# MpokiAbel/UPMEM--OpenFHE

Hardware: AMD Instinct MI355X
Metric: 64-bit coeffs/sec for NTT+Hadamard+INTT, N=2^16, 16 towers; % HBM roofline (higher is better)
Workload: dtype u64; 1 GPU; configs[2]: N=2^16, towers=16, batch=1024 per GPU, c = INTT(NTT(a) (.) b); log_n=16, towers=16, batch_per_gpu=1024, global_batch=1024, parallelism=batch-sharded x1 (no data-path collective)

## Files before the change

### upmem--openfhe_amd/csrc/ntt_kernels.hpp

```cpp
#pragma once
#include "arith.hpp"

namespace ofhe {

struct TowerConst {
    u64 q;
    u64 ninv;
    u64 ninv_pre;
    u64 mu;
    u64 nq;
    u64 nq4;
    u32 nshift;
    u32 spq_sh;
    u64 qinv;
    u32 one;
    u32 pad_;
};
template <bool SPQ>
__device__ __forceinline__ Mod<SPQ> load_mod(const TowerConst& tc) {
    return Mod<SPQ>{tc.q, 4 * tc.q, 8 * tc.q, tc.nq, tc.nq4, 0 - 8 * tc.q, tc.spq_sh, tc.one};
}

struct PlanArgs {
    const TowerConst* tc;
    const u64* tw;
    const u64* itw;
    const u64* tw3;
    u64 sstride;
    u64 dstride;
    u64 bstride;
    const u64* scal;
    const u64* dtw;
    const u64* twist;
    u32 log_n;
    u32 towers;
};

enum { MODE_FWD = 0, MODE_INV = 1, MODE_FUSED = 2, MODE_FWD_SUB = 3 };

__device__ __forceinline__ u32 xcd_remap(u32 bid, u32 nwg) {
    u32 q = nwg >> 3, r = nwg & 7, xcd = bid & 7, loc = bid >> 3;
    return (xcd < r ? xcd * (q + 1) : r * (q + 1) + (xcd - r) * q) + loc;
}

struct Tw {
    u64 w, wp;
};

typedef u64 u64x2 __attribute__((ext_vector_type(2)));
__device__ __forceinline__ u64 ld_s(const u64* p) { return __builtin_nontemporal_load(p); }
__device__ __forceinline__ void st_s(u64* p, u64 v) { __builtin_nontemporal_store(v, p); }
__device__ __forceinline__ u64x2 ld2_s(const u64* p) {
    return __builtin_nontemporal_load(reinterpret_cast<const u64x2*>(p));
}
__device__ __forceinline__ void st2_s(u64* p, u64x2 v) { __builtin_nontemporal_store(v, reinterpret_cast<u64x2*>(p)); }
__device__ __forceinline__ Tw ldtw(const u64* base, u32 idx) {
    const ulonglong2 v = *reinterpret_cast<const ulonglong2*>(base + 2 * (u64)idx);
    return Tw{v.x, v.y};
}

template <bool SPQ, bool QA>
__device__ __forceinline__ u64 red16(u64 x, const Mod<SPQ, QA>& M) {
    if (SPQ) return fold_spq(x, M);
    return csub_s(x, M.q8);
}
template <bool SPQ, bool QA>
__device__ __forceinline__ void ct_bfly_cs(u64& x, u64& y, Tw w, const Mod<SPQ, QA>& M, bool cs) {
    const u64 a = cs ? red16(x, M) : x;
    x = shoup_lazy_acc(y, w.w, w.wp, M, a);
    y = (a << 1) + M.q4 - x;
}
template <int CS, class M_>
__device__ __forceinline__ void ct_bfly(u64& x, u64& y, Tw w, const M_& M) {
    ct_bfly_cs(x, y, w, M, CS != 0);
}

template <bool SPQ, bool QA>
__device__ __forceinline__ u64 red8(u64 x, const Mod<SPQ, QA>& M) {
    return csub_s(x, M.q4);
}
template <bool SPQ, bool QA>
__device__ __forceinline__ u64 red16_gs(u64 x, const Mod<SPQ, QA>& M) {
    return csub_s(x, M.q8);
}

template <class M_>
__device__ __forceinline__ void gs_bfly(u64& x, u64& y, Tw w, const M_& M) {
    const u64 s = x + y;
    const u64 d = x + M.q4 - y;
    x = red8(s, M);
    y = shoup_lazy(d, w.w, w.wp, M);
}

__device__ __forceinline__ u64 canon8(u64 x, u64 q) {
    x = csub_s(x, 4 * q);
    x = csub_s(x, 2 * q);
    return csub_s(x, q);
}
__device__ __forceinline__ u64 canon4(u64 x, u64 q) {
    x = csub_s(x, 2 * q);
    return csub_s(x, q);
}
template <bool SPQ, bool QA>
__device__ __forceinline__ u64 canon_spq(u64 x, const Mod<SPQ, QA>& M) {
    const u32 qh = hi32(x) >> M.sh;
    const u64 d = (1ull << (M.sh + 32)) - M.q;
    const u64 xm = pack(lo32(x), hi32(x) & ((1u << M.sh) - 1));
    return csub_s(mad32(qh, lo32(d), xm), M.q);
}
template <bool SPQ, bool QA>
__device__ __forceinline__ u64 canon8m(u64 x, const Mod<SPQ, QA>& M) {
    return SPQ ? canon_spq(x, M) : canon8(x, M.q);
}
template <bool SPQ, bool QA>
__device__ __forceinline__ u64 canon4m(u64 x, const Mod<SPQ, QA>& M) {
    return SPQ ? canon_spq(x, M) : canon4(x, M.q);
}
template <bool SPQ, bool QA>
__device__ __forceinline__ u64 canon_fwd(u64 x, const Mod<SPQ, QA>& M) {
    if (SPQ) return canon_spq(x, M);
    const u64 q = M.q;
    x = csub_s(x, 8 * q);
    return canon8(x, q);
}


__device__ __forceinline__ void triv_bfly(u64& x, u64& y, u64 bq) {
    const u64 s = x + y;
    y = x + bq - y;
    x = s;
}

template <int H, int CS, class M_>
__device__ __forceinline__ void dit_stage16(u64 (&v)[16], const u64* base, u32 st, const M_& M) {
    constexpr int half = 1 << H;
#pragma unroll
    for (int j = 0; j < half; j++) {
        const Tw w = ldtw(base, st * j);
#pragma unroll
        for (int g = 0; g < 16; g += 2 * half) ct_bfly<CS>(v[g + j], v[g + j + half], w, M);
    }
}
template <class M_>
__device__ __forceinline__ void dit_round16(u64 (&v)[16], const u64* dtw, u32 st, u32 r, const M_& M) {
    dit_stage16<0, 1>(v, dtw + 2 * ((u64)st + r), st, M);
    dit_stage16<1, 0>(v, dtw + 2 * ((u64)2 * st + r), st, M);
    dit_stage16<2, 1>(v, dtw + 2 * ((u64)4 * st + r), st, M);
    dit_stage16<3, 0>(v, dtw + 2 * ((u64)8 * st + r), st, M);
}

template <bool SPQ, bool QA>
__device__ __forceinline__ void dit_round3(u64 (&v)[16], const u64* dtw, const Mod<SPQ, QA>& M) {
#pragma unroll
    for (int g = 0; g < 16; g += 2) triv_bfly(v[g], v[g + 1], 2 * M.q);
#pragma unroll
    for (int g = 0; g < 16; g += 4) triv_bfly(v[g], v[g + 2], M.q4);
    {
        const Tw w = ldtw(dtw, 3);
#pragma unroll
        for (int g = 0; g < 16; g += 4) ct_bfly<0>(v[g + 1], v[g + 3], w, M);
    }
#pragma unroll
    for (int g = 0; g < 16; g += 8) triv_bfly(v[g], v[g + 4], M.q8);
#pragma unroll
    for (int j = 1; j < 4; j++) {
        const Tw w = ldtw(dtw, 4 + j);
#pragma unroll
        for (int g = 0; g < 16; g += 8) ct_bfly<0>(v[g + j], v[g + j + 4], w, M);
    }
    {
        const u64 a = red16(v[0], M), b = red16(v[8], M);
        v[0] = a;
        v[8] = b;
        triv_bfly(v[0], v[8], M.q8);
    }
#pragma unroll
    for (int j = 1; j < 8; j++) ct_bfly<1>(v[j], v[j + 8], ldtw(dtw, 8 + j), M);
}

template <bool SPQ, bool QA>
__device__ __forceinline__ u64 twist_out(u64 x, Tw f, const Mod<SPQ, QA>& M) {
    return canon4m(shoup_lazy(x, f.w, f.wp, M), M);
}

template <int S, class M_, int CS = S & 1>
__device__ __forceinline__ void fwd_stage16(u64 (&v)[16], const u64* tw, u32 M0, const M_& M) {
    constexpr int half = 8 >> S;
    const u64* base = tw + 2 * ((u64)M0 << S);
#pragma unroll
    for (int j = 0; j < (1 << S); j++) {
        Tw w = ldtw(base, j);
#pragma unroll
        for (int k = j * 2 * half; k < j * 2 * half + half; k++) ct_bfly<CS>(v[k], v[k + half], w, M);
    }
}

template <int S, class M_>
__device__ __forceinline__ void inv_stage16(u64 (&v)[16], const u64* itw, u32 M0, const M_& M) {
    constexpr int half = 8 >> S;
    const u64* base = itw + 2 * ((u64)M0 << S);
#pragma unroll
    for (int j = 0; j < (1 << S); j++) {
        Tw w = ldtw(base, j);
#pragma unroll
        for (int k = j * 2 * half; k < j * 2 * half + half; k++) gs_bfly(v[k], v[k + half], w, M);
    }
}

template <class M_>
__device__ __forceinline__ void gs_bfly_b(u64& x, u64& y, Tw w, const M_& M, bool in8) {
    const u64 s = x + y;
    const u64 d = x + (in8 ? M.q8 : M.q4) - y;
    x = in8 ? red16_gs(s, M) : s;
    y = shoup_lazy(d, w.w, w.wp, M);
}
template <int S, class M_>
__device__ __forceinline__ void inv_stage16_b(u64 (&v)[16], bool (&b8)[16], const u64* itw, u32 M0, const M_& M) {
    constexpr int half = 8 >> S;
    const u64* base = itw + 2 * ((u64)M0 << S);
#pragma unroll
    for (int j = 0; j < (1 << S); j++) {
        Tw w = ldtw(base, j);
#pragma unroll
        for (int k = j * 2 * half; k < j * 2 * half + half; k++) {
            gs_bfly_b(v[k], v[k + half], w, M, b8[k] || b8[k + half]);
            b8[k] = true;
            b8[k + half] = false;
        }
    }
}
template <class M_>
__device__ __forceinline__ void inv_round16_b(u64 (&v)[16], bool (&b8)[16], const u64* itw, u32 M0, const M_& M) {
    inv_stage16_b<3>(v, b8, itw, M0, M);
    inv_stage16_b<2>(v, b8, itw, M0, M);
    inv_stage16_b<1>(v, b8, itw, M0, M);
    inv_stage16_b<0>(v, b8, itw, M0, M);
}

template <class M_>
__device__ __forceinline__ void fwd_round16(u64 (&v)[16], const u64* tw, u32 M0, const M_& M) {
    fwd_stage16<0>(v, tw, M0, M);
    fwd_stage16<1>(v, tw, M0, M);
    fwd_stage16<2>(v, tw, M0, M);
    fwd_stage16<3>(v, tw, M0, M);
}
template <class M_>
__device__ __forceinline__ void fwd_round16_canon(u64 (&v)[16], const u64* tw, u32 M0, const M_& M) {
    fwd_stage16<0>(v, tw, M0, M);
    fwd_stage16<1, M_, 0>(v, tw, M0, M);
    fwd_stage16<2>(v, tw, M0, M);
    fwd_stage16<3>(v, tw, M0, M);
}
template <class M_>
__device__ __forceinline__ void inv_round16(u64 (&v)[16], const u64* itw, u32 M0, const M_& M) {
    inv_stage16<3>(v, itw, M0, M);
    inv_stage16<2>(v, itw, M0, M);
    inv_stage16<1>(v, itw, M0, M);
    inv_stage16<0>(v, itw, M0, M);
}

template <int S, class M_>
__device__ __forceinline__ void fwd_stage16_t3(u64 (&v)[16], const u64* tw3, u32 U, u32 u, const M_& M) {
    constexpr int half = 8 >> S;
    const u64* base = tw3 + 2 * (u64)(((1u << S) - 1) * U);
#pragma unroll
    for (int j = 0; j < (1 << S); j++) {
        Tw w = ldtw(base + 2 * (u64)j * U, u);
#pragma unroll
        for (int k = j * 2 * half; k < j * 2 * half + half; k++) ct_bfly<S & 1>(v[k], v[k + half], w, M);
    }
}
__device__ __forceinline__ u32 lds_pad(u32 p) { return p + (p >> 4); }
constexpr u32 LDS_WORDS = 4096 + 4096 / 16;

template <bool TEAM>
struct StageMap {
    u32 l, base;
    static constexpr u32 E = TEAM ? 32 : 128;
    __device__ __forceinline__ explicit StageMap(u32 tid)
        : l(TEAM ? (tid & 15) : (tid & 63)), base(TEAM ? (tid >> 4) * 256 : (tid >> 6) * 1024) {}
    __device__ __forceinline__ u32 g(int k) const { return E * k + 2 * l; }
    __device__ __forceinline__ u32 p(int k) const { return lds_pad(base + g(k)); }
};
template <bool TEAM>
__device__ __forceinline__ void wave_stage_in(const u64* wsrc, u64* lds, u32 tid, u64 (&out)[16]) {
    const StageMap<TEAM> m(tid);
#pragma unroll
    for (int k = 0; k < 8; k++) {
        const u64x2 v = ld2_s(wsrc + m.g(k));
        lds[m.p(k)] = v.x;
        lds[m.p(k) + 1] = v.y;
    }
    __builtin_amdgcn_wave_barrier();
#pragma unroll
    for (int k = 0; k < 16; k++) out[k] = lds[tid * 17 + k];
    __builtin_amdgcn_wave_barrier();
}
template <bool TEAM, int NPRE>
__device__ __forceinline__ void wave_stage_in_pre(const u64* wsrc, u64* lds, u32 tid, const u64x2 (&pre)[NPRE > 0 ? NPRE : 1],
                                                  u64 (&out)[16]) {
    const StageMap<TEAM> m(tid);
#pragma unroll
    for (int k = 0; k < 8; k++) {
        const u64x2 v = k < NPRE ? pre[k < NPRE ? k : 0] : ld2_s(wsrc + m.g(k));
        lds[m.p(k)] = v.x;
        lds[m.p(k) + 1] = v.y;
    }
    __builtin_amdgcn_wave_barrier();
#pragma unroll
    for (int k = 0; k < 16; k++) out[k] = lds[tid * 17 + k];
    __builtin_amdgcn_wave_barrier();
}
template <bool TEAM>
__device__ __forceinline__ void wave_stage_out(const u64 (&v)[16], u64* lds, u32 tid, u64* wdst, bool live = true) {
    const StageMap<TEAM> m(tid);
#pragma unroll
    for (int k = 0; k < 16; k++) lds[tid * 17 + k] = v[k];
    __builtin_amdgcn_wave_barrier();
    u64x2 w[8];
#pragma unroll
    for (int k = 0; k < 8; k++) {
        w[k].x = lds[m.p(k)];
        w[k].y = lds[m.p(k) + 1];
    }
    if (live) {
#pragma unroll
        for (int k = 0; k < 8; k++) st2_s(wdst + m.g(k), w[k]);
    }
}

#ifndef OFHE_B_PF
#define OFHE_B_PF 8
#endif
#ifndef OFHE_KB_WAVES
#define OFHE_KB_WAVES 4
#endif
template <int NR>
__device__ __forceinline__ void block_sync() {
    if (NR == 2)
        __builtin_amdgcn_wave_barrier();
    else
        __syncthreads();
}
template <int MODE, bool SPQ, int NR, int SK = 0>
__device__ __forceinline__ void block_body(const PlanArgs& P, const u64* src, u64* dst, const u64* __restrict__ bdat,
                                           u32 batch, u32 wid, u64* lds, u32 tid) {
    static_assert(NR == 2 || NR == 3, "k_block covers the last 8 (NR=2) or 12 (NR=3) stages");
    static_assert(SK == 0 || (SK == 3 && NR == 3), "k_block: SK = 3 needs NR = 3");
    constexpr bool TEAM = NR == 2;
    const u32 logn = P.log_n;
    const u32 N = 1u << logn;
    const u32 h = tid >> 4, r = tid & 15;
    u32 g, t, b;
    bool live = true;
    if (TEAM) {
        const u32 G4 = N >> 10, nq = (batch + 3) >> 2;
        const u32 wave = __builtin_amdgcn_readfirstlane(tid >> 6);
        g = (wid % G4) * 4 + wave;
        const u32 pq = wid / G4;
        t = pq / nq;
        const u32 bt = (pq % nq) * 4 + (h & 3);
        live = bt < batch;
        b = live ? bt : batch - 1;
    } else {
        const u32 G = N >> 12;
        g = wid % G;
        const u32 pb = wid / G;
        t = pb / batch;
        b = pb % batch;
    }
    const u64 inner = (u64)t * N + ((u64)g << (TEAM ? 8 : 12));
    const u64 off = (u64)b * P.dstride + inner;
    const u64 boff = (u64)b * P.bstride + inner;
    const u32 wq = TEAM ? 0 : (tid >> 6) * 1024;
    const u64* blk = src + (u64)b * P.sstride + inner;
    u64* oblk = dst + off;
    const TowerConst tc = P.tc[t];
    const u64 q = tc.q;
    const Mod<SPQ> M = load_mod<SPQ>(tc);
    const u64* tw = P.tw + (u64)t * N * 2;
    const u32 L1 = tid + h;
    const u32 L2 = h * 272 + r;
    const u32 L3 = tid * 17;
    u64 v[16];

    if (MODE == MODE_FWD || MODE == MODE_FUSED || MODE == MODE_FWD_SUB) {
        if (NR == 3) {
#pragma unroll
            for (int k = 0; k < 16; k++) v[k] = ld_s(blk + tid + 256 * k);
            if (SK == 3)
                fwd_stage16<3>(v, tw, (N >> 12) + g, M);
            else
                fwd_round16(v, tw, (N >> 12) + g, M);
#pragma unroll
            for (int k = 0; k < 16; k++) lds[L1 + 272 * k] = v[k];
            __syncthreads();
#pragma unroll
            for (int k = 0; k < 16; k++) v[k] = lds[L2 + 17 * k];
        } else {
#pragma unroll
            for (int k = 0; k < 16; k++) v[k] = ld_s(blk + r + 16 * k);
        }
        fwd_round16(v, tw, (N >> 8) + (TEAM ? g : g * 16 + h), M);
#pragma unroll
        for (int k = 0; k < 16; k++) lds[L2 + 17 * k] = v[k];
        block_sync<NR>();
#pragma unroll
        for (int k = 0; k < 16; k++) v[k] = lds[L3 + k];
        constexpr int BPF = (MODE == MODE_FUSED || MODE == MODE_FWD_SUB) ? OFHE_B_PF : 0;
        u64x2 bpre[BPF > 0 ? BPF : 1];
#pragma unroll
        for (int k = 0; k < BPF; k++) bpre[k] = ld2_s(bdat + boff + wq + StageMap<TEAM>(tid).g(k));
        {
            const u64* tw3 = P.tw3 + (u64)t * (N / 16) * 30;
            const u32 U = N >> 4, u = TEAM ? g * 16 + r : g * 256 + tid;
            fwd_stage16_t3<0>(v, tw3, U, u, M);
            fwd_stage16_t3<1>(v, tw3, U, u, M);
            fwd_stage16_t3<2>(v, tw3, U, u, M);
            fwd_stage16_t3<3>(v, tw3, U, u, M);
        }
        if (MODE == MODE_FWD) {
#pragma unroll
            for (int k = 0; k < 16; k++) v[k] = canon_fwd<SPQ>(v[k], M);
            wave_stage_out<TEAM>(v, lds, tid, oblk + wq, live);
            return;
        }
        if (MODE == MODE_FWD_SUB) {
            u64 xx[16];
            wave_stage_in_pre<TEAM, BPF>(bdat + boff + wq, lds, tid, bpre, xx);
            const u64 sc = P.scal[3 * t + 1], scp = P.scal[3 * t + 2];
            const u64 q12 = M.q8 + M.q4;
#pragma unroll
            for (int k = 0; k < 16; k++) v[k] = canon4m(shoup_lazy(xx[k] + q12 - v[k], sc, scp, M), M);
            wave_stage_out<TEAM>(v, lds, tid, oblk + wq, live);
            return;
        }
        u64 bb[16];
        wave_stage_in_pre<TEAM, BPF>(bdat + boff + wq, lds, tid, bpre, bb);
#pragma unroll
        for (int k = 0; k < 16; k++) v[k] = mont_mul(v[k], bb[k], q, tc.qinv);
    } else {
        wave_stage_in<TEAM>(blk + wq, lds, tid, v);
    }
    const u64* dtw = P.dtw + (u64)t * N * 2;
    dit_round3(v, dtw, M);
#pragma unroll
    for (int k = 0; k < 16; k++) lds[L3 + k] = v[k];
    block_sync<NR>();
#pragma unroll
    for (int k = 0; k < 16; k++) v[k] = lds[L2 + 17 * k];
    dit_round16(v, dtw, 16, r, M);
    const u64* tw_ = P.twist + (u64)t * N * 2 + 2 * ((u64)g << (TEAM ? 8 : 12));
    if (NR == 2) {
#pragma unroll
        for (int k = 0; k < 16; k++) {
            const Tw f = ldtw(tw_, r + 16 * k);
            v[k] = shoup_lazy(v[k], f.w, f.wp, M);
        }
        if (live) {
#pragma unroll
            for (int k = 0; k < 16; k++) st_s(oblk + r + 16 * k, v[k]);
        }
        return;
    }
#pragma unroll
    for (int k = 0; k < 16; k++) lds[L2 + 17 * k] = v[k];
    __syncthreads();
#pragma unroll
    for (int k = 0; k < 16; k++) v[k] = lds[L1 + 272 * k];
    if (SK == 3)
        dit_stage16<0, 1>(v, dtw + 2 * ((u64)256 + tid), 256, M);
    else
        dit_round16(v, dtw, 256, tid, M);
#pragma unroll
    for (int k = 0; k < 16; k++) {
        const Tw f = ldtw(tw_, tid + 256 * k);
        v[k] = logn == 12 ? twist_out(v[k], f, M) : shoup_lazy(v[k], f.w, f.wp, M);
    }
#pragma unroll
    for (int k = 0; k < 16; k++) st_s(oblk + tid + 256 * k, v[k]);
}
template <int MODE, bool SPQ, int NR, int SK = 0>
__global__ __launch_bounds__(256, OFHE_KB_WAVES) void k_block(PlanArgs P, const u64* src, u64* dst,
                                                              const u64* __restrict__ bdat, u32 batch, u32 nwg) {
    OFHE_VGPR_FLOOR();
    __shared__ u64 lds[LDS_WORDS];
    block_body<MODE, SPQ, NR, SK>(P, src, dst, bdat, batch, xcd_remap(blockIdx.x, nwg), lds, threadIdx.x);
}

struct SwSrc {
    const u64* last;
    u64 lstride;
    u64 ql;
    const u64* tab;
    u64 pre, pre_p;
};
#ifndef OFHE_TCOLS_W
#define OFHE_TCOLS_W 16
#endif
constexpr u32 TCOLS_W = OFHE_TCOLS_W;
static_assert(TCOLS_W == 16 || TCOLS_W == 32, "column tile width");
constexpr u32 TCOLS_LDS_WORDS = 16 * 16 * TCOLS_W + 16 * 16;
template <bool INV, bool SPQ, bool SWS = false, int LOGN = 16>
__device__ __forceinline__ void tcols_body(const PlanArgs& P, const u64* src, u64* dst, u32 batch, u32 wid,
                                           const SwSrc& SWA, u64* lds, u32 tid) {
    static_assert(LOGN == 16 || LOGN == 17, "k_tcols: N = 2^16 or 2^17");
    constexpr u32 N = 1u << LOGN, S = N / 256, W = TCOLS_W;
    const u32 cb = wid % (S / W);
    const u32 pb = wid / (S / W);
    const u32 t = pb / batch, b = pb % batch;
    const u64 inner = (u64)t * N + cb * W;
    const u64* x = src + (u64)b * P.sstride + inner;
    u64* y = dst + (u64)b * P.dstride + inner;
    const TowerConst tc = P.tc[t];
    const Mod<SPQ> M = load_mod<SPQ>(tc);
    const u32 h = tid / W, r = tid % W;
    const u32 L1 = tid, L2 = h * 16 * W + r;
    u64 v[16];
    if (!INV) {
        const u64* tw = P.tw + (u64)t * N * 2;
        constexpr u32 RP = 16 * W + 16;
        if (SWS) {
            const u64 w = SWA.tab[6 * t + 1], wp = SWA.tab[6 * t + 2];
            const SwMod sm = sw_mod(SWA.ql, tc.q);
            const u64* lp = SWA.last + (u64)b * SWA.lstride + cb * W;
#pragma unroll
            for (int k = 0; k < 16; k++) {
                u64 e = lp[(u64)(h + 16 * k) * S + r];
                if (SWA.pre != 1) e = shoup_canon(e, SWA.pre, SWA.pre_p, SWA.ql);
                e = switch_mod1(e, sm);
                v[k] = w != 1 ? shoup_canon(e, w, wp, tc.q) : e;
            }
        } else {
#pragma unroll
            for (int k = 0; k < 16; k++) v[k] = ld_s(x + (u64)(h + 16 * k) * S + r);
        }
        fwd_round16_canon(v, tw, 1, M);
#pragma unroll
        for (int k = 0; k < 16; k++) lds[L1 + RP * k] = v[k];
        __syncthreads();
#pragma unroll
        for (int k = 0; k < 16; k++) v[k] = lds[h * RP + r + W * k];
        fwd_round16(v, tw, 16 + h, M);
#pragma unroll
        for (int k = 0; k < 16; k++) st_s(y + (u64)(16 * h + k) * S + r, v[k]);
    } else {
        const u64* itw = P.itw + (u64)t * N * 2;
#pragma unroll
        for (int k = 0; k < 16; k++) v[k] = ld_s(x + (u64)(16 * h + k) * S + r);
        bool b8[16];
#pragma unroll
        for (int k = 0; k < 16; k++) b8[k] = false;
        inv_round16_b(v, b8, itw, 16 + h, M);
#pragma unroll
        for (int k = 0; k < 16; k++) lds[L2 + W * k] = v[k];
        __syncthreads();
#pragma unroll
        for (int k = 0; k < 16; k++) {
            v[k] = lds[L1 + 16 * W * k];
            b8[k] = true;
        }
        inv_round16_b(v, b8, itw, 1, M);
#pragma unroll
        for (int k = 0; k < 16; k++)
            st_s(y + (u64)(h + 16 * k) * S + r, b8[k] ? canon8m(v[k], M) : canon4m(v[k], M));
    }
}

template <bool INV, bool SPQ, bool SWS = false, int LOGN = 16>
__global__ __launch_bounds__(16 * TCOLS_W, OFHE_KB_WAVES) void k_tcols(PlanArgs P, const u64* src, u64* dst, u32 batch,
                                                                       u32 nwg, SwSrc SWA) {
    OFHE_VGPR_FLOOR();
    __shared__ u64 lds[TCOLS_LDS_WORDS];
    tcols_body<INV, SPQ, SWS, LOGN>(P, src, dst, batch, xcd_remap(blockIdx.x, nwg), SWA, lds, threadIdx.x);
}

template <bool INV, bool SPQ>
__global__ __launch_bounds__(512) void k_tcols9(PlanArgs P, const u64* src, u64* dst, u32 batch, u32 nwg) {
    OFHE_VGPR_FLOOR();
    constexpr u32 N = 1u << 17, S = 256, W = 16, HALF = 16 * 16 * W;
    __shared__ u64 lds[2 * HALF];
    const u32 tid = threadIdx.x;
    const u32 hf = tid >> 8, tl = tid & 255;
    const u32 wid = xcd_remap(blockIdx.x, nwg);
    const u32 cb = wid % (S / W);
    const u32 pb = wid / (S / W);
    const u32 t = pb / batch, b = pb % batch;
    const u64 inner = (u64)t * N + (u64)hf * 256 * S + cb * W;
    const u64* x = src + (u64)b * P.sstride + inner;
    u64* y = dst + (u64)b * P.dstride + inner;
    const TowerConst tc = P.tc[t];
    const Mod<SPQ> M = load_mod<SPQ>(tc);
    const u32 h = tl / W, r = tl % W;
    u64* my = lds + hf * HALF;
    const u64* other = lds + (hf ^ 1) * HALF;
    const u32 L1 = tl, L2 = h * 16 * W + r;
    u64 v[16];
    if (!INV) {
        const u64* tw = P.tw + (u64)t * N * 2;
#pragma unroll
        for (int k = 0; k < 16; k++) v[k] = ld_s(x + (u64)(h + 16 * k) * S + r);
        const Tw w1 = ldtw(tw, 1);
        if (hf) {
#pragma unroll
            for (int k = 0; k < 16; k++) v[k] = shoup_lazy(v[k], w1.w, w1.wp, M);
        }
#pragma unroll
        for (int k = 0; k < 16; k++) my[L1 + 16 * W * k] = v[k];
        __syncthreads();
        if (hf) {
#pragma unroll
            for (int k = 0; k < 16; k++) v[k] = other[L1 + 16 * W * k] + M.q4 - v[k];
        } else {
#pragma unroll
            for (int k = 0; k < 16; k++) v[k] += other[L1 + 16 * W * k];
        }
        __syncthreads();
        fwd_round16(v, tw, 2 + hf, M);
#pragma unroll
        for (int k = 0; k < 16; k++) my[L1 + 16 * W * k] = v[k];
        __syncthreads();
#pragma unroll
        for (int k = 0; k < 16; k++) v[k] = my[L2 + W * k];
        fwd_round16(v, tw, 32 + 16 * hf + h, M);
#pragma unroll
        for (int k = 0; k < 16; k++) st_s(y + (u64)(16 * h + k) * S + r, v[k]);
    } else {
        const u64* itw = P.itw + (u64)t * N * 2;
#pragma unroll
        for (int k = 0; k < 16; k++) v[k] = ld_s(x + (u64)(16 * h + k) * S + r);
        inv_round16(v, itw, 32 + 16 * hf + h, M);
#pragma unroll
        for (int k = 0; k < 16; k++) my[L2 + W * k] = v[k];
        __syncthreads();
#pragma unroll
        for (int k = 0; k < 16; k++) v[k] = my[L1 + 16 * W * k];
        inv_round16(v, itw, 2 + hf, M);
#pragma unroll
        for (int k = 0; k < 16; k++) my[L1 + 16 * W * k] = v[k];
        __syncthreads();
// ... 184 lines not shown
```

### upmem--openfhe_amd/csrc/ofhe_hip.hip

```cpp
#include <cstdio>
#include <cstdlib>
#include <cstring>
#include <new>
#include <thread>

#include "compose.hpp"
#include "bconv_cols.hpp"

using namespace ofhe;

#define OFHE_VERSION "ofhe-hip 0.2 gfx950"

namespace ofhe {
static thread_local std::string g_err;
int fail(int code, const std::string& msg) {
    g_err = msg;
    return code;
}
int post_launch() {
    hipError_t e = hipGetLastError();
    if (e != hipSuccess) return fail(OFHE_ERR_HIP, std::string("kernel launch: ") + hipGetErrorString(e));
    return OFHE_OK;
}
}
// ... 348 lines not shown
                  {(void**)&p->d_itw, itw.data(), words(itw)},
                  {(void**)&p->d_tw3, tw3.data(), words(tw3)},
                  {(void**)&p->d_dtw, dtw.data(), words(dtw)},
                  {(void**)&p->d_twist, twist.data(), words(twist)},
                  {(void**)&p->d_twist_r, twist_r.data(), words(twist_r)}};
    int rc = OFHE_OK;
    for (const auto& t : tables)
        if (rc == OFHE_OK) rc = alloc_upload(t.dst, t.src, t.bytes, "plan upload", ctx->device);
    if (rc != OFHE_OK) {
        ofhe_hip_plan_destroy(p);
        return rc;
    }
    *plan = p;
    return OFHE_OK;
}

int ofhe_hip_plan_tune(ofhe_plan_t p, uint32_t chunk_batch, uint32_t streams) {
    if (!p || !p->ctx) return fail(OFHE_ERR_STATE, "plan is NULL or destroyed");
    if (streams < 1 || streams > 2) return fail(OFHE_ERR_ARG, "streams must be 1 or 2");
    HIPCHK(hipSetDevice(p->ctx->device));
    std::lock_guard<std::mutex> lk(p->fork_mu);
    if (streams == 2 && !p->st[0]) {
        hipStream_t st[2] = {nullptr, nullptr};
        hipEvent_t fork = nullptr, join[2] = {nullptr, nullptr};
        hipError_t e = hipSuccess;
        for (int i = 0; i < 2 && e == hipSuccess; i++) {
            e = hipStreamCreateWithFlags(&st[i], hipStreamNonBlocking);
            if (e == hipSuccess) e = hipEventCreateWithFlags(&join[i], hipEventDisableTiming);
        }
        if (e == hipSuccess) e = hipEventCreateWithFlags(&fork, hipEventDisableTiming);
        if (e != hipSuccess) {
            for (int i = 0; i < 2; i++) {
                if (st[i]) (void)hipStreamDestroy(st[i]);
                if (join[i]) (void)hipEventDestroy(join[i]);
            }
            if (fork) (void)hipEventDestroy(fork);
            return fail(OFHE_ERR_HIP, std::string("plan_tune: ") + hipGetErrorString(e));
        }
        for (int i = 0; i < 2; i++) {
            p->st[i] = st[i];
            p->ev_join[i] = join[i];
        }
        p->ev_fork = fork;
    }
    p->chunk_batch = chunk_batch;
    p->nstreams = streams;
    return OFHE_OK;
}

int ofhe_hip_plan_destroy(ofhe_plan_t p) {
    if (!p) return fail(OFHE_ERR_ARG, "plan is NULL");
    if (p->ctx) (void)hipSetDevice(p->ctx->device);
    for (int i = 0; i < 2; i++) {
        if (p->st[i]) (void)hipStreamSynchronize(p->st[i]);
        if (p->st[i]) (void)hipStreamDestroy(p->st[i]);
        if (p->ev_join[i]) (void)hipEventDestroy(p->ev_join[i]);
    }
    if (p->ev_fork) (void)hipEventDestroy(p->ev_fork);
    (void)hipFree(p->d_tc);
    (void)hipFree(p->d_tw);
    (void)hipFree(p->d_itw);
    (void)hipFree(p->d_tw3);
    (void)hipFree(p->d_dtw);
    (void)hipFree(p->d_twist);
    (void)hipFree(p->d_twist_r);
    for (auto& kv : p->tabs) (void)hipFree(kv.second);
    delete p;
    return OFHE_OK;
}

int ofhe_hip_plan_tables(ofhe_plan_t p, uint64_t* tab, uint64_t* tab_pre, uint64_t* itab,
                         uint64_t* itab_pre, uint64_t* ninv) {
    if (!p) return fail(OFHE_ERR_ARG, "plan is NULL");
    const size_t n = p->tab.size() * sizeof(u64);
    if (tab) memcpy(tab, p->tab.data(), n);
    if (tab_pre) memcpy(tab_pre, p->tab_pre.data(), n);
    if (itab) memcpy(itab, p->itab.data(), n);
    if (itab_pre) memcpy(itab_pre, p->itab_pre.data(), n);
    if (ninv) memcpy(ninv, p->ninv.data(), p->ninv.size() * sizeof(u64));
    return OFHE_OK;
}

static PlanArgs args_of(ofhe_plan_t p, u32 t0 = 0, u32 count = 0) {
    if (!count) count = p->towers - t0;
    const u64 N = 1ull << p->log_n;
    PlanArgs a;
    a.tc = p->d_tc + t0;
    a.tw = p->d_tw + 2 * N * t0;
    a.itw = p->d_itw + 2 * N * t0;
    a.tw3 = p->d_tw3 + (N >= 4096 ? (N / 16) * 30 * t0 : 0);
    a.sstride = a.dstride = a.bstride = N * count;
    a.scal = nullptr;
    a.dtw = p->d_dtw + 2 * N * t0;
    a.twist = p->d_twist + 2 * N * t0;
    a.log_n = p->log_n;
    a.towers = count;
    return a;
}

static PlanArgs fused_args(ofhe_plan_t p) {
    PlanArgs a = args_of(p);
    if (p->log_n >= 12) a.twist = p->d_twist_r;
    return a;
}

static int check_common(ofhe_plan_t p, uint32_t batch) {
    if (!p || !p->ctx) return fail(OFHE_ERR_STATE, "plan is NULL or destroyed");
    if (batch == 0) return fail(OFHE_ERR_ARG, "batch must be >= 1");
    const u64 polys = (u64)batch * p->towers;
    if (polys * ((u64)1 << p->log_n) / 4096 >= (1ull << 31))
        return fail(OFHE_ERR_ARG, "batch too large for one launch");
    return OFHE_OK;
}

#ifndef OFHE_COLS_CPT
#define OFHE_COLS_CPT 2
#endif
static void launch_colpass(const PlanArgs& a, bool spq, int split, bool inv, const u64* src, u64* dst, u32 batch,
                           hipStream_t s, const SwSrc* lift = nullptr) {
    const SwSrc S = lift ? *lift : SwSrc{nullptr, 0, 0, nullptr, 1, 0};
    const u32 polys = batch * a.towers;
    with_bool(spq, [&](auto sp) { with_bool(inv, [&](auto iv) { with_bool(lift != nullptr, [&](auto sw) {
        constexpr bool SP = decltype(sp)::value, INV = decltype(iv)::value, SWS = decltype(sw)::value;
        if constexpr (!(INV && SWS)) {
            if (split == SPLIT_T9) {
                if constexpr (!SWS) {
                    const u32 nwg = polys * 16;
                    hipLaunchKernelGGL((k_tcols9<INV, SP>), dim3(nwg), dim3(512), 0, s, a, src, dst, batch, nwg);
                }
            } else if (split != SPLIT_COLS) {
                with_int<16, 17>(split == SPLIT_T8B9 ? 17 : 16, [&](auto ln) {
                    constexpr int LOGN = decltype(ln)::value;
                    const u32 nwg = polys * ((1u << (LOGN - 8)) / TCOLS_W);
                    hipLaunchKernelGGL((k_tcols<INV, SP, SWS, LOGN>), dim3(nwg), dim3(16 * TCOLS_W), 0, s, a, src,
                                       dst, batch, nwg, S);
                });
            } else {
                with_int<1, 2, 3, 4, 5>((int)a.log_n - 12, [&](auto ka) {
                    constexpr int KA = decltype(ka)::value, CPT = KA <= 4 ? OFHE_COLS_CPT : 1;
                    const u32 nwg = polys * (16 / CPT);
                    hipLaunchKernelGGL((k_cols<KA, INV, CPT, SP, SWS>), dim3(nwg), dim3(256), 0, s, a, src, dst,
                                       batch, nwg, S);
                });
            }
        }
    }); }); });
}

template <int MODE>
static void launch_block(const PlanArgs& a, bool spq, const u64* src, u64* dst, const u64* b, u32 batch,
                         hipStream_t s, int split = SPLIT_COLS) {
    with_bool(spq, [&](auto sp) { with_int<8, 9, 12>((int)block_stages(split, a.log_n), [&](auto st) {
        constexpr int NR = decltype(st)::value == 8 ? 2 : 3, SK = decltype(st)::value == 9 ? 3 : 0;
        const u32 nwg = NR == 2 ? ((batch + 3) / 4) * a.towers * (1u << (a.log_n - 10))
                                : batch * a.towers * (1u << (a.log_n - 12));
        hipLaunchKernelGGL((k_block<MODE, decltype(sp)::value, NR, SK>), dim3(nwg), dim3(256), 0, s, a, src, dst, b,
                           batch, nwg);
    }); });
}

template <int MODE>
static void launch_small(const PlanArgs& a, bool spq, const u64* src, u64* dst, const u64* b, u32 batch,
                         hipStream_t s) {
    const u32 N = 1u << a.log_n;
    const u32 thr = N / 2 >= 256 ? 256 : (N / 2 < 64 ? 64 : N / 2);
    with_bool(spq, [&](auto sp) {
        hipLaunchKernelGGL((k_small<MODE, decltype(sp)::value>), dim3(batch * a.towers), dim3(thr), 0, s, a, src, dst,
                           b, batch);
    });
}


namespace ofhe {
int plan_ntt_range(ofhe_plan_t p, bool inverse, u32 t0, u32 count, const u64* src, u64* dst, u64 sstride,
                   u64 dstride, u32 batch, hipStream_t s) {
    if (!p || !p->ctx) return fail(OFHE_ERR_STATE, "plan is NULL or destroyed");
    if (count == 0 || batch == 0) return OFHE_OK;
    if (t0 + count > p->towers || t0 + count < t0) return fail(OFHE_ERR_ARG, "tower range outside the plan");
    if (!src || !dst) return fail(OFHE_ERR_ARG, "data is NULL");
    const u64 N = 1ull << p->log_n;
    if (sstride < N * count || dstride < N * count)
        return fail(OFHE_ERR_ARG, "batch stride smaller than the tower range");
    if ((u64)batch * count * N / 4096 >= (1ull << 31)) return fail(OFHE_ERR_ARG, "batch too large for one launch");
    HIPCHK(hipSetDevice(p->ctx->device));
    PlanArgs a = args_of(p, t0, count);
    PlanArgs ad = a;
    a.sstride = sstride;
    a.dstride = ad.sstride = ad.dstride = dstride;
    if (!inverse) {
        if (p->log_n < 12) {
            launch_small<MODE_FWD>(a, p->spq, src, dst, nullptr, batch, s);
        } else if (p->log_n == 12) {
            launch_block<MODE_FWD>(a, p->spq, src, dst, nullptr, batch, s, p->split);
        } else {
            launch_colpass(a, p->spq, p->split, false, src, dst, batch, s);
            launch_block<MODE_FWD>(ad, p->spq, dst, dst, nullptr, batch, s, p->split);
        }
    } else {
        if (p->log_n < 12) {
            launch_small<MODE_INV>(a, p->spq, src, dst, nullptr, batch, s);
        } else {
            launch_block<MODE_INV>(a, p->spq, src, dst, nullptr, batch, s, p->split);
            if (p->log_n > 12) launch_colpass(ad, p->spq, p->split, true, dst, dst, batch, s);
        }
    }
    return post_launch();
}

int plan_cols_switch(ofhe_plan_t p, u32 t0, u32 count, const u64* last, u64 lstride, u64 ql, u64 pre, const u64* tab,
                     u64* y, u64 ystride, u32 batch, hipStream_t s) {
    if (!p || !p->ctx) return fail(OFHE_ERR_STATE, "plan is NULL or destroyed");
    if (p->log_n <= 12 || p->split == SPLIT_T9) return fail(OFHE_ERR_ARG, "plan_cols_switch: k_cols / k_tcols plans only");
    if (((uintptr_t)last & 15) || (lstride & 1)) return fail(OFHE_ERR_ARG, "plan_cols_switch: misaligned source");
    HIPCHK(hipSetDevice(p->ctx->device));
    PlanArgs a = args_of(p, t0, count);
    a.sstride = a.dstride = ystride;
    pre %= ql;
    const SwSrc S{last, lstride, ql, tab, pre, pre == 1 ? 0 : shoup_pre(pre, ql)};
    launch_colpass(a, p->spq, p->split, false, nullptr, y, batch, s, &S);
    return post_launch();
}

int plan_ntt_fwd_block(ofhe_plan_t p, u32 t0, u32 count, u64* y, u64 ystride, u32 batch, hipStream_t s) {
    if (!p || !p->ctx) return fail(OFHE_ERR_STATE, "plan is NULL or destroyed");
    if (p->log_n <= 12) return fail(OFHE_ERR_ARG, "plan_ntt_fwd_block: log_n > 12 only");
    HIPCHK(hipSetDevice(p->ctx->device));
    PlanArgs a = args_of(p, t0, count);
    a.sstride = a.dstride = ystride;
    launch_block<MODE_FWD>(a, p->spq, y, y, nullptr, batch, s, p->split);
    return post_launch();
}

int plan_ntt_inv_block(ofhe_plan_t p, u32 t0, u32 count, const u64* src, u64 sstride, u64* dst, u64 dstride, u32 batch,
                       hipStream_t s) {
    if (!p || !p->ctx) return fail(OFHE_ERR_STATE, "plan is NULL or destroyed");
    if (p->log_n <= 12) return fail(OFHE_ERR_ARG, "plan_ntt_inv_block: log_n > 12 only");
    if (count == 0 || batch == 0) return OFHE_OK;
    if (t0 + count > p->towers) return fail(OFHE_ERR_ARG, "tower range outside the plan");
    HIPCHK(hipSetDevice(p->ctx->device));
    PlanArgs a = args_of(p, t0, count);
    a.sstride = sstride;
    a.dstride = dstride;
    launch_block<MODE_INV>(a, p->spq, src, dst, nullptr, batch, s, p->split);
    return post_launch();
}

int plan_ntt_fwd_sub(ofhe_plan_t p, u32 t0, u32 count, u64* y, u64 ystride, const u64* x, u64 xstride, u64* out,
                     u64 ostride, const u64* scal, u32 batch, hipStream_t s, int parts) {
    if (!p || !p->ctx) return fail(OFHE_ERR_STATE, "plan is NULL or destroyed");
    if (p->log_n < 12) return fail(OFHE_ERR_ARG, "fused forward + subtract needs log_n >= 12");
    if (count == 0 || batch == 0) return OFHE_OK;
    if (t0 + count > p->towers) return fail(OFHE_ERR_ARG, "tower range outside the plan");
    HIPCHK(hipSetDevice(p->ctx->device));
    PlanArgs a = args_of(p, t0, count);
    a.sstride = a.dstride = ystride;
    if (p->log_n > 12 && (parts & 1)) launch_colpass(a, p->spq, p->split, false, y, y, batch, s);
    if (!(parts & 2)) return post_launch();
    PlanArgs ab = a;
    ab.sstride = ystride;
    ab.dstride = ostride;
    ab.bstride = xstride;
    ab.scal = scal;
    launch_block<MODE_FWD_SUB>(ab, p->spq, y, out, x, batch, s, p->split);
    return post_launch();
}
}

int ofhe_hip_ntt_fwd(ofhe_plan_t p, uint64_t* data, uint32_t batch, void* stream) {
    RCCHK(check_common(p, batch));
    if (!data) return fail(OFHE_ERR_ARG, "data is NULL");
    const u64 d = (u64)p->towers << p->log_n;
    return plan_ntt_range(p, false, 0, p->towers, data, data, d, d, batch, pick(stream));
}

int ofhe_hip_ntt_inv(ofhe_plan_t p, uint64_t* data, uint32_t batch, void* stream) {
    RCCHK(check_common(p, batch));
    if (!data) return fail(OFHE_ERR_ARG, "data is NULL");
    const u64 d = (u64)p->towers << p->log_n;
    return plan_ntt_range(p, true, 0, p->towers, data, data, d, d, batch, pick(stream));
}

int ofhe_hip_ntt_fwd_range(ofhe_plan_t p, uint32_t t0, uint32_t count, const uint64_t* src, uint64_t* dst,
                           uint64_t src_stride, uint64_t dst_stride, uint32_t batch, void* stream) {
    if (!p || !p->ctx) return fail(OFHE_ERR_STATE, "plan is NULL or destroyed");
    if (batch == 0 || count == 0) return fail(OFHE_ERR_ARG, "batch and count must be >= 1");
    return plan_ntt_range(p, false, t0, count, src, dst, src_stride, dst_stride, batch, pick(stream));
}

int ofhe_hip_ntt_inv_range(ofhe_plan_t p, uint32_t t0, uint32_t count, const uint64_t* src, uint64_t* dst,
                           uint64_t src_stride, uint64_t dst_stride, uint32_t batch, void* stream) {
    if (!p || !p->ctx) return fail(OFHE_ERR_STATE, "plan is NULL or destroyed");
    if (batch == 0 || count == 0) return fail(OFHE_ERR_ARG, "batch and count must be >= 1");
    return plan_ntt_range(p, true, t0, count, src, dst, src_stride, dst_stride, batch, pick(stream));
}

int ofhe_hip_ntt_mul_intt(ofhe_plan_t p, const uint64_t* a_, const uint64_t* b, uint64_t* c,
                          uint32_t batch, void* stream) {
    int rc = check_common(p, batch);
    if (rc) return rc;
    if (!a_ || !b || !c) return fail(OFHE_ERR_ARG, "NULL data pointer");
    if (b == c && a_ != c) return fail(OFHE_ERR_ARG, "c may alias a but not b");
    HIPCHK(hipSetDevice(p->ctx->device));
    const PlanArgs a = fused_args(p);
    hipStream_t s = pick(stream);
    if (p->log_n < 12) {
        launch_small<MODE_FUSED>(a, p->spq, a_, c, b, batch, s);
    } else if (p->log_n == 12) {
        launch_block<MODE_FUSED>(a, p->spq, a_, c, b, batch, s, p->split);
    } else {
        const u32 cb = (p->chunk_batch && p->chunk_batch < batch) ? p->chunk_batch : batch;
// ... 448 lines not shown
```

Before: 85.34 billion coeffs/s.

## Remap NR=2 block kernel to share column group across batch, cache twiddles in LDS

In the NR=2 team path, a workgroup now covers one 256-point column group for 16 batch entries instead of four column groups for four batch entries. Because every wave uses the same twiddles, the workgroup loads twist, tw3 and DIT twiddle tables into LDS once. A full __syncthreads then replaces the wave barrier, and the inner stages read twiddles from LDS rather than global memory. This cuts global twiddle traffic at the cost of extra LDS, a block-wide barrier and a different work decomposition.

```diff
diff --git a/upmem--openfhe_amd/csrc/ntt_kernels.hpp b/upmem--openfhe_amd/csrc/ntt_kernels.hpp
--- a/upmem--openfhe_amd/csrc/ntt_kernels.hpp
+++ b/upmem--openfhe_amd/csrc/ntt_kernels.hpp
@@ -1,4 +1,6 @@
 #pragma once
+#include <type_traits>
+
 #include "arith.hpp"
 
 namespace ofhe {
@@ -335,12 +337,49 @@
 #ifndef OFHE_KB_WAVES
 #define OFHE_KB_WAVES 4
 #endif
+#ifndef OFHE_WG16_TAB
+#define OFHE_WG16_TAB 10
+#endif
 template <int NR>
 __device__ __forceinline__ void block_sync() {
     if (NR == 2)
         __builtin_amdgcn_wave_barrier();
     else
         __syncthreads();
+}
+template <int MODE, int NR>
+struct BlockTabs {
+    static constexpr bool FWDP = MODE != MODE_INV, INVP = MODE == MODE_INV || MODE == MODE_FUSED;
+    static constexpr bool TWIST = NR == 2 && INVP && (OFHE_WG16_TAB & 1);
+    static constexpr bool TW3 = NR == 2 && FWDP && (OFHE_WG16_TAB & 2);
+    static constexpr bool DIT = NR == 2 && INVP && (OFHE_WG16_TAB & 4);
+    static constexpr bool DIT8 = NR == 2 && INVP && !DIT && (OFHE_WG16_TAB & 8);
+    static constexpr bool ANY = TWIST || TW3 || DIT || DIT8;
+    static constexpr u32 O_TWIST = LDS_WORDS, O_TW3 = O_TWIST + (TWIST ? 512 : 0), O_DIT = O_TW3 + (TW3 ? 512 : 0);
+    static constexpr u32 WORDS = O_DIT + (DIT ? 512 : DIT8 ? 256 : 0);
+};
+template <u32 WORDS>
+struct alignas(16) LdsTabBuf {
+    u64 w[WORDS];
+};
+template <int MODE, int NR>
+using BlockLds = std::conditional_t<BlockTabs<MODE, NR>::ANY, LdsTabBuf<BlockTabs<MODE, NR>::WORDS>, u64[LDS_WORDS]>;
+template <u32 WORDS>
+__device__ __forceinline__ u64* lds_words(LdsTabBuf<WORDS>& b) { return b.w; }
+__device__ __forceinline__ u64* lds_words(u64 (&b)[LDS_WORDS]) { return b; }
+__device__ __forceinline__ ulonglong2 ldtab(const u64* base, u32 slot) {
+    return *reinterpret_cast<const ulonglong2*>(base + 2 * (u64)slot);
+}
+__device__ __forceinline__ void sttab(u64* tab, u32 slot, ulonglong2 v) {
+    *reinterpret_cast<ulonglong2*>(tab + 2 * slot) = v;
+}
+template <class TB>
+__device__ __forceinline__ void tabs_publish(u64* lds, u32 tid, ulonglong2 f_twist, ulonglong2 f_tw3, ulonglong2 f_dit) {
+    if (TB::TWIST) sttab(lds + TB::O_TWIST, tid, f_twist);
+    if (TB::TW3) sttab(lds + TB::O_TW3, tid, f_tw3);
+    if (TB::DIT) sttab(lds + TB::O_DIT, tid, f_dit);
+    if (TB::DIT8 && tid >= 128) sttab(lds + TB::O_DIT, tid - 128, f_dit);
+    __syncthreads();
 }
 template <int MODE, bool SPQ, int NR, int SK = 0>
 __device__ __forceinline__ void block_body(const PlanArgs& P, const u64* src, u64* dst, const u64* __restrict__ bdat,
@@ -354,12 +393,11 @@
     u32 g, t, b;
     bool live = true;
     if (TEAM) {
-        const u32 G4 = N >> 10, nq = (batch + 3) >> 2;
-        const u32 wave = __builtin_amdgcn_readfirstlane(tid >> 6);
-        g = (wid % G4) * 4 + wave;
-        const u32 pq = wid / G4;
-        t = pq / nq;
-        const u32 bt = (pq % nq) * 4 + (h & 3);
+        const u32 G = N >> 8, nb = (batch + 15) >> 4;
+        g = wid % G;
+        const u32 pq = wid / G;
+        t = pq / nb;
+        const u32 bt = (pq % nb) * 16 + h;
         live = bt < batch;
         b = live ? bt : batch - 1;
     } else {
@@ -383,6 +421,11 @@
     const u32 L2 = h * 272 + r;
     const u32 L3 = tid * 17;
     u64 v[16];
+    using TB = BlockTabs<MODE, NR>;
+    ulonglong2 f_twist = {}, f_tw3 = {}, f_dit = {};
+    if (TB::TWIST) f_twist = ldtab(P.twist + (u64)t * N * 2 + 2 * ((u64)g << 8), tid);
+    if (TB::TW3) f_tw3 = ldtab(P.tw3 + (u64)t * (N / 16) * 30, (h < 15 ? h : 14) * (N >> 4) + g * 16 + r);
+    if (TB::DIT || (TB::DIT8 && tid >= 128)) f_dit = ldtab(P.dtw + (u64)t * N * 2, tid);
 
     if (MODE == MODE_FWD || MODE == MODE_FUSED || MODE == MODE_FWD_SUB) {
         if (NR == 3) {
@@ -404,7 +447,10 @@
         fwd_round16(v, tw, (N >> 8) + (TEAM ? g : g * 16 + h), M);
 #pragma unroll
         for (int k = 0; k < 16; k++) lds[L2 + 17 * k] = v[k];
-        block_sync<NR>();
+        if (TB::ANY)
+            tabs_publish<TB>(lds, tid, f_twist, f_tw3, f_dit);
+        else
+            block_sync<NR>();
 #pragma unroll
         for (int k = 0; k < 16; k++) v[k] = lds[L3 + k];
         constexpr int BPF = (MODE == MODE_FUSED || MODE == MODE_FWD_SUB) ? OFHE_B_PF : 0;
@@ -412,8 +458,8 @@
 #pragma unroll
         for (int k = 0; k < BPF; k++) bpre[k] = ld2_s(bdat + boff + wq + StageMap<TEAM>(tid).g(k));
         {
-            const u64* tw3 = P.tw3 + (u64)t * (N / 16) * 30;
-            const u32 U = N >> 4, u = TEAM ? g * 16 + r : g * 256 + tid;
+            const u64* tw3 = TB::TW3 ? lds + TB::O_TW3 : P.tw3 + (u64)t * (N / 16) * 30;
+            const u32 U = TB::TW3 ? 16 : N >> 4, u = TB::TW3 ? r : TEAM ? g * 16 + r : g * 256 + tid;
             fwd_stage16_t3<0>(v, tw3, U, u, M);
             fwd_stage16_t3<1>(v, tw3, U, u, M);
             fwd_stage16_t3<2>(v, tw3, U, u, M);
@@ -446,11 +492,21 @@
     dit_round3(v, dtw, M);
 #pragma unroll
     for (int k = 0; k < 16; k++) lds[L3 + k] = v[k];
-    block_sync<NR>();
+    if (TB::ANY && MODE == MODE_INV)
+        tabs_publish<TB>(lds, tid, f_twist, f_tw3, f_dit);
+    else
+        block_sync<NR>();
 #pragma unroll
     for (int k = 0; k < 16; k++) v[k] = lds[L2 + 17 * k];
-    dit_round16(v, dtw, 16, r, M);
-    const u64* tw_ = P.twist + (u64)t * N * 2 + 2 * ((u64)g << (TEAM ? 8 : 12));
+    if (TB::DIT8) {
+        dit_stage16<0, 1>(v, dtw + 2 * ((u64)16 + r), 16, M);
+        dit_stage16<1, 0>(v, dtw + 2 * ((u64)32 + r), 16, M);
+        dit_stage16<2, 1>(v, dtw + 2 * ((u64)64 + r), 16, M);
+        dit_stage16<3, 0>(v, lds + TB::O_DIT + 2 * r, 16, M);
+    } else {
+        dit_round16(v, TB::DIT ? lds + TB::O_DIT : dtw, 16, r, M);
+    }
+    const u64* tw_ = TB::TWIST ? lds + TB::O_TWIST : P.twist + (u64)t * N * 2 + 2 * ((u64)g << (TEAM ? 8 : 12));
     if (NR == 2) {
 #pragma unroll
         for (int k = 0; k < 16; k++) {
@@ -484,8 +540,8 @@
 __global__ __launch_bounds__(256, OFHE_KB_WAVES) void k_block(PlanArgs P, const u64* src, u64* dst,
                                                               const u64* __restrict__ bdat, u32 batch, u32 nwg) {
     OFHE_VGPR_FLOOR();
-    __shared__ u64 lds[LDS_WORDS];
-    block_body<MODE, SPQ, NR, SK>(P, src, dst, bdat, batch, xcd_remap(blockIdx.x, nwg), lds, threadIdx.x);
+    __shared__ BlockLds<MODE, NR> lds;
+    block_body<MODE, SPQ, NR, SK>(P, src, dst, bdat, batch, xcd_remap(blockIdx.x, nwg), lds_words(lds), threadIdx.x);
 }
 
 struct SwSrc {
diff --git a/upmem--openfhe_amd/csrc/ofhe_hip.hip b/upmem--openfhe_amd/csrc/ofhe_hip.hip
--- a/upmem--openfhe_amd/csrc/ofhe_hip.hip
+++ b/upmem--openfhe_amd/csrc/ofhe_hip.hip
@@ -524,7 +524,7 @@
                          hipStream_t s, int split = SPLIT_COLS) {
     with_bool(spq, [&](auto sp) { with_int<8, 9, 12>((int)block_stages(split, a.log_n), [&](auto st) {
         constexpr int NR = decltype(st)::value == 8 ? 2 : 3, SK = decltype(st)::value == 9 ? 3 : 0;
-        const u32 nwg = NR == 2 ? ((batch + 3) / 4) * a.towers * (1u << (a.log_n - 10))
+        const u32 nwg = NR == 2 ? ((batch + 15) / 16) * a.towers * (1u << (a.log_n - 8))
                                 : batch * a.towers * (1u << (a.log_n - 12));
         hipLaunchKernelGGL((k_block<MODE, decltype(sp)::value, NR, SK>), dim3(nwg), dim3(256), 0, s, a, src, dst, b,
                            batch, nwg);
```

After: 84.21 billion coeffs/s. -1.3%, worse.

## Process two polynomials per thread in fused block pass to reuse twiddles

Applied to the files above, without the earlier changes.

Adds a QP=2 variant of the fused NR=2 block kernel for log_n=16. Each thread keeps two batch polynomials in registers and applies every loaded twiddle to both, which halves twiddle loads per coefficient and halves the grid size. In exchange it doubles register pressure, and launch bounds drop to 3 waves, which may lower occupancy and latency hiding.

```diff
diff --git a/upmem--openfhe_amd/csrc/ntt_kernels.hpp b/upmem--openfhe_amd/csrc/ntt_kernels.hpp
--- a/upmem--openfhe_amd/csrc/ntt_kernels.hpp
+++ b/upmem--openfhe_amd/csrc/ntt_kernels.hpp
@@ -270,6 +270,101 @@
         for (int k = j * 2 * half; k < j * 2 * half + half; k++) ct_bfly<S & 1>(v[k], v[k + half], w, M);
     }
 }
+template <int S, int Q, class M_>
+__device__ __forceinline__ void fwd_stage16(u64 (&v)[Q][16], const u64* tw, u32 M0, const M_& M) {
+    constexpr int half = 8 >> S;
+    const u64* base = tw + 2 * ((u64)M0 << S);
+#pragma unroll
+    for (int j = 0; j < (1 << S); j++) {
+        Tw w = ldtw(base, j);
+#pragma unroll
+        for (int k = j * 2 * half; k < j * 2 * half + half; k++)
+#pragma unroll
+            for (int c = 0; c < Q; c++) ct_bfly<S & 1>(v[c][k], v[c][k + half], w, M);
+    }
+}
+template <int Q, class M_>
+__device__ __forceinline__ void fwd_round16(u64 (&v)[Q][16], const u64* tw, u32 M0, const M_& M) {
+    fwd_stage16<0>(v, tw, M0, M);
+    fwd_stage16<1>(v, tw, M0, M);
+    fwd_stage16<2>(v, tw, M0, M);
+    fwd_stage16<3>(v, tw, M0, M);
+}
+template <int S, int Q, class M_>
+__device__ __forceinline__ void fwd_stage16_t3(u64 (&v)[Q][16], const u64* tw3, u32 U, u32 u, const M_& M) {
+    constexpr int half = 8 >> S;
+    const u64* base = tw3 + 2 * (u64)(((1u << S) - 1) * U);
+#pragma unroll
+    for (int j = 0; j < (1 << S); j++) {
+        Tw w = ldtw(base + 2 * (u64)j * U, u);
+#pragma unroll
+        for (int k = j * 2 * half; k < j * 2 * half + half; k++)
+#pragma unroll
+            for (int c = 0; c < Q; c++) ct_bfly<S & 1>(v[c][k], v[c][k + half], w, M);
+    }
+}
+template <int H, int CS, int Q, class M_>
+__device__ __forceinline__ void dit_stage16(u64 (&v)[Q][16], const u64* base, u32 st, const M_& M) {
+    constexpr int half = 1 << H;
+#pragma unroll
+    for (int j = 0; j < half; j++) {
+        const Tw w = ldtw(base, st * j);
+#pragma unroll
+        for (int g = 0; g < 16; g += 2 * half)
+#pragma unroll
+            for (int c = 0; c < Q; c++) ct_bfly<CS>(v[c][g + j], v[c][g + j + half], w, M);
+    }
+}
+template <int Q, class M_>
+__device__ __forceinline__ void dit_round16(u64 (&v)[Q][16], const u64* dtw, u32 st, u32 r, const M_& M) {
+    dit_stage16<0, 1>(v, dtw + 2 * ((u64)st + r), st, M);
+    dit_stage16<1, 0>(v, dtw + 2 * ((u64)2 * st + r), st, M);
+    dit_stage16<2, 1>(v, dtw + 2 * ((u64)4 * st + r), st, M);
+    dit_stage16<3, 0>(v, dtw + 2 * ((u64)8 * st + r), st, M);
+}
+template <int Q, bool SPQ, bool QA>
+__device__ __forceinline__ void dit_round3(u64 (&v)[Q][16], const u64* dtw, const Mod<SPQ, QA>& M) {
+#pragma unroll
+    for (int c = 0; c < Q; c++) {
+#pragma unroll
+        for (int g = 0; g < 16; g += 2) triv_bfly(v[c][g], v[c][g + 1], 2 * M.q);
+#pragma unroll
+        for (int g = 0; g < 16; g += 4) triv_bfly(v[c][g], v[c][g + 2], M.q4);
+    }
+    {
+        const Tw w = ldtw(dtw, 3);
+#pragma unroll
+        for (int g = 0; g < 16; g += 4)
+#pragma unroll
+            for (int c = 0; c < Q; c++) ct_bfly<0>(v[c][g + 1], v[c][g + 3], w, M);
+    }
+#pragma unroll
+    for (int c = 0; c < Q; c++)
+#pragma unroll
+        for (int g = 0; g < 16; g += 8) triv_bfly(v[c][g], v[c][g + 4], M.q8);
+#pragma unroll
+    for (int j = 1; j < 4; j++) {
+        const Tw w = ldtw(dtw, 4 + j);
+#pragma unroll
+        for (int g = 0; g < 16; g += 8)
+#pragma unroll
+            for (int c = 0; c < Q; c++) ct_bfly<0>(v[c][g + j], v[c][g + j + 4], w, M);
+    }
+#pragma unroll
+    for (int c = 0; c < Q; c++) {
+        const u64 a = red16(v[c][0], M), b = red16(v[c][8], M);
+        v[c][0] = a;
+        v[c][8] = b;
+        triv_bfly(v[c][0], v[c][8], M.q8);
+    }
+#pragma unroll
+    for (int j = 1; j < 8; j++) {
+        const Tw w = ldtw(dtw, 8 + j);
+#pragma unroll
+        for (int c = 0; c < Q; c++) ct_bfly<1>(v[c][j], v[c][j + 8], w, M);
+    }
+}
+
 __device__ __forceinline__ u32 lds_pad(u32 p) { return p + (p >> 4); }
 constexpr u32 LDS_WORDS = 4096 + 4096 / 16;
 
@@ -480,12 +575,116 @@
 #pragma unroll
     for (int k = 0; k < 16; k++) st_s(oblk + tid + 256 * k, v[k]);
 }
-template <int MODE, bool SPQ, int NR, int SK = 0>
-__global__ __launch_bounds__(256, OFHE_KB_WAVES) void k_block(PlanArgs P, const u64* src, u64* dst,
-                                                              const u64* __restrict__ bdat, u32 batch, u32 nwg) {
+template <bool SPQ>
+__device__ __forceinline__ void block_body_q2(const PlanArgs& P, const u64* src, u64* dst,
+                                              const u64* __restrict__ bdat, u32 batch, u32 wid, u64* lds, u32 tid) {
+    constexpr int QP = 2;
+    const u32 N = 1u << P.log_n;
+    const u32 h = tid >> 4, r = tid & 15;
+    const u32 G4 = N >> 10, no = (batch + 7) >> 3;
+    const u32 wave = __builtin_amdgcn_readfirstlane(tid >> 6);
+    const u32 g = (wid % G4) * 4 + wave;
+    const u32 po = wid / G4;
+    const u32 t = po / no;
+    const u64 inner = (u64)t * N + ((u64)g << 8);
+    bool live[QP];
+    u64 boff[QP];
+    const u64* blk[QP];
+    u64* oblk[QP];
+#pragma unroll
+    for (int s = 0; s < QP; s++) {
+        const u32 bt = (po % no) * 8 + 4 * s + (h & 3);
+        live[s] = bt < batch;
+        const u32 b = live[s] ? bt : batch - 1;
+        boff[s] = (u64)b * P.bstride + inner;
+        blk[s] = src + (u64)b * P.sstride + inner;
+        oblk[s] = dst + ((u64)b * P.dstride + inner);
+    }
+    const TowerConst tc = P.tc[t];
+    const u64 q = tc.q;
+    const Mod<SPQ> M = load_mod<SPQ>(tc);
+    const u64* tw = P.tw + (u64)t * N * 2;
+    const u32 L2 = h * 272 + r;
+    const u32 L3 = tid * 17;
+    u64 v[QP][16];
+
+#pragma unroll
+    for (int s = 0; s < QP; s++)
+#pragma unroll
+        for (int k = 0; k < 16; k++) v[s][k] = ld_s(blk[s] + r + 16 * k);
+    fwd_round16(v, tw, (N >> 8) + g, M);
+#pragma unroll
+    for (int s = 0; s < QP; s++) {
+#pragma unroll
+        for (int k = 0; k < 16; k++) lds[L2 + 17 * k] = v[s][k];
+        __builtin_amdgcn_wave_barrier();
+#pragma unroll
+        for (int k = 0; k < 16; k++) v[s][k] = lds[L3 + k];
+        __builtin_amdgcn_wave_barrier();
+    }
+    constexpr int BPF = SPQ ? OFHE_B_PF : 3;
+    u64x2 bpre[QP][BPF > 0 ? BPF : 1];
+#pragma unroll
+    for (int s = 0; s < QP; s++)
+#pragma unroll
+        for (int k = 0; k < BPF; k++) bpre[s][k] = ld2_s(bdat + boff[s] + StageMap<true>(tid).g(k));
+    {
+        const u64* tw3 = P.tw3 + (u64)t * (N / 16) * 30;
+        const u32 U = N >> 4, u = g * 16 + r;
+        fwd_stage16_t3<0>(v, tw3, U, u, M);
+        fwd_stage16_t3<1>(v, tw3, U, u, M);
+        fwd_stage16_t3<2>(v, tw3, U, u, M);
+        fwd_stage16_t3<3>(v, tw3, U, u, M);
+    }
+#pragma unroll
+    for (int s = 0; s < QP; s++) {
+        u64 bb[16];
+        wave_stage_in_pre<true, BPF>(bdat + boff[s], lds, tid, bpre[s], bb);
+#pragma unroll
+        for (int k = 0; k < 16; k++) v[s][k] = mont_mul(v[s][k], bb[k], q, tc.qinv);
+    }
+    const u64* dtw = P.dtw + (u64)t * N * 2;
+    dit_round3(v, dtw, M);
+#pragma unroll
+    for (int s = 0; s < QP; s++) {
+#pragma unroll
+        for (int k = 0; k < 16; k++) lds[L3 + k] = v[s][k];
+        __builtin_amdgcn_wave_barrier();
+#pragma unroll
+        for (int k = 0; k < 16; k++) v[s][k] = lds[L2 + 17 * k];
+        __builtin_amdgcn_wave_barrier();
+    }
+    dit_round16(v, dtw, 16, r, M);
+    const u64* tw_ = P.twist + (u64)t * N * 2 + 2 * ((u64)g << 8);
+    constexpr int TG = 4;
+#pragma unroll
+    for (int k0 = 0; k0 < 16; k0 += TG) {
+#pragma unroll
+        for (int k = k0; k < k0 + TG; k++) {
+            const Tw f = ldtw(tw_, r + 16 * k);
+#pragma unroll
+            for (int s = 0; s < QP; s++) v[s][k] = shoup_lazy(v[s][k], f.w, f.wp, M);
+        }
+#pragma unroll
+        for (int s = 0; s < QP; s++) {
+            if (live[s]) {
+#pragma unroll
+                for (int k = k0; k < k0 + TG; k++) st_s(oblk[s] + r + 16 * k, v[s][k]);
+            }
+        }
+    }
+}
+template <int MODE, bool SPQ, int NR, int SK = 0, int QP = 1>
+__global__ __launch_bounds__(256, QP == 2 ? 3 : OFHE_KB_WAVES) void k_block(PlanArgs P, const u64* src, u64* dst,
+                                                                            const u64* __restrict__ bdat, u32 batch,
+                                                                            u32 nwg) {
+    static_assert(QP == 1 || (QP == 2 && NR == 2 && MODE == MODE_FUSED), "k_block: QP = 2 is the fused NR = 2 pass");
     OFHE_VGPR_FLOOR();
     __shared__ u64 lds[LDS_WORDS];
-    block_body<MODE, SPQ, NR, SK>(P, src, dst, bdat, batch, xcd_remap(blockIdx.x, nwg), lds, threadIdx.x);
+    if constexpr (QP == 2)
+        block_body_q2<SPQ>(P, src, dst, bdat, batch, xcd_remap(blockIdx.x, nwg), lds, threadIdx.x);
+    else
+        block_body<MODE, SPQ, NR, SK>(P, src, dst, bdat, batch, xcd_remap(blockIdx.x, nwg), lds, threadIdx.x);
 }
 
 struct SwSrc {
diff --git a/upmem--openfhe_amd/csrc/ofhe_hip.hip b/upmem--openfhe_amd/csrc/ofhe_hip.hip
--- a/upmem--openfhe_amd/csrc/ofhe_hip.hip
+++ b/upmem--openfhe_amd/csrc/ofhe_hip.hip
@@ -524,10 +524,13 @@
                          hipStream_t s, int split = SPLIT_COLS) {
     with_bool(spq, [&](auto sp) { with_int<8, 9, 12>((int)block_stages(split, a.log_n), [&](auto st) {
         constexpr int NR = decltype(st)::value == 8 ? 2 : 3, SK = decltype(st)::value == 9 ? 3 : 0;
-        const u32 nwg = NR == 2 ? ((batch + 3) / 4) * a.towers * (1u << (a.log_n - 10))
-                                : batch * a.towers * (1u << (a.log_n - 12));
-        hipLaunchKernelGGL((k_block<MODE, decltype(sp)::value, NR, SK>), dim3(nwg), dim3(256), 0, s, a, src, dst, b,
-                           batch, nwg);
+        with_bool(NR == 2 && MODE == MODE_FUSED && a.log_n == 16, [&](auto oct) {
+            constexpr int QP = (NR == 2 && MODE == MODE_FUSED && decltype(oct)::value) ? 2 : 1;
+            const u32 nwg = NR == 2 ? ((batch + 4 * QP - 1) / (4 * QP)) * a.towers * (1u << (a.log_n - 10))
+                                    : batch * a.towers * (1u << (a.log_n - 12));
+            hipLaunchKernelGGL((k_block<MODE, decltype(sp)::value, NR, SK, QP>), dim3(nwg), dim3(256), 0, s, a, src,
+                               dst, b, batch, nwg);
+        });
     }); });
 }
 
```

After: 81.89 billion coeffs/s before, 82.75 billion coeffs/s after (median of 6 runs). 1.1% higher.
